# TUMFTM/RadarGNN

Measured on AMD Instinct MI355X. Metric: radar frames/sec (graph-build + GNN fwd), higher is better.
Workload: dtype f32 (dense layers: fp32 operands split into 2 f16 terms after an exact power-of-two pre-scale, 3 f16 MFMA products per fp32 product, fp32 accumulate -- more accurate than fp32 MFMA against float64, tests/test_gpu_f16x2.py; RGNN_NO_F16X2=1 selects 3 bf16 terms / 6 products, RGNN_LINEAR_FP32=1 v_mfma_; 1 GPU; C2: per GPU 64 RadarScenes-shaped frames x 3000 pts, radius graph r=1.0, node feats [rcs,velocity_vector,time_index,degree], edge feats [relative_position], 4-layer MPNNConv [224,224,128,64] + emb MLPs + both heads, train-mode BatchNorm, max aggr; frames_per_gpu=64, points_per_gpu=192000, edges_per_gpu=799078, ranks_in_process_group=1

## Files before the change

radargnn_amd/csrc/mpnn_tiles.hip:

```cpp
#include "common.h"
#include <stdlib.h>
#include <type_traits>

namespace {

constexpr int MT_THREADS = 256;
constexpr int MT_WAVES = MT_THREADS / 64;
constexpr int MT_QUEUE_INTS = 8 * 16;

typedef float mt_f32x16 __attribute__((ext_vector_type(16)));
typedef __bf16 mt_bf16x8 __attribute__((ext_vector_type(8)));
typedef unsigned int mt_u32x4 __attribute__((ext_vector_type(4)));

__global__ __launch_bounds__(256) void k_tiles_zero_empty(const int32_t* __restrict__ rowptr, const int32_t* __restrict__ order,
                                                         int64_t n, int d, float* __restrict__ out, int64_t ldo) {
  const int lane = threadIdx.x & 63;
  const int64_t p = (int64_t)blockIdx.x * MT_WAVES + (threadIdx.x >> 6);
  if (p >= n || rowptr[p + 1] != rowptr[p]) return;
  const int64_t node = order ? order[p] : p;
  for (int c = lane; c < d; c += 64) out[node * ldo + c] = 0.f;
}

__device__ __forceinline__ void mt_split3(float x, unsigned& t1, unsigned& t2, unsigned& t3) {
  t1 = __float_as_uint(x) & 0xffff0000u;
  const float r = x - __uint_as_float(t1);
  t2 = __float_as_uint(r) & 0xffff0000u;
  const float r2 = r - __uint_as_float(t2);
  t3 = __float_as_uint(r2) & 0xffff0000u;
}
__device__ __forceinline__ unsigned mt_pack(unsigned lo, unsigned hi) { return (lo >> 16) | hi; }
__device__ __forceinline__ void mt_split_row(const float (&x)[8], mt_u32x4& p1, mt_u32x4& p2, mt_u32x4& p3) {
  unsigned t1[8], t2[8], t3[8];
#pragma unroll
  for (int k = 0; k < 8; k++) mt_split3(x[k], t1[k], t2[k], t3[k]);
  p1 = mt_u32x4{mt_pack(t1[0], t1[1]), mt_pack(t1[2], t1[3]), mt_pack(t1[4], t1[5]), mt_pack(t1[6], t1[7])};
  p2 = mt_u32x4{mt_pack(t2[0], t2[1]), mt_pack(t2[2], t2[3]), mt_pack(t2[4], t2[5]), mt_pack(t2[6], t2[7])};
  p3 = mt_u32x4{mt_pack(t3[0], t3[1]), mt_pack(t3[2], t3[3]), mt_pack(t3[4], t3[5]), mt_pack(t3[6], t3[7])};
}

}

namespace {

constexpr int WN_SLOTS = 512;
constexpr int WN_THREADS = 256;
typedef int wn_i32x4 __attribute__((ext_vector_type(4)));

struct WinParams {
  const float* p_bias;
  const float* Q; int ldq4; int q_bytes;
  const mt_u32x4* wplanes;
  const float* ea; int de; int ea_vec;
  int n_win;
  const int32_t* n_win_dev;
  const int32_t* plan; int plan_bytes;
  int off_misc;
  int off_eid;
  int off_lrow;
  int off_urow;
  int off_tgt;
  int32_t* queue;
  int d; int n_ct;
  float* out; int ldo4; int o_bytes;
  float* out_absmax;
  int abl;
};

__device__ __forceinline__ void wn_dma16(wn_i32x4 rsrc, int voff, int soff, unsigned lds_base) {
  asm volatile(
      "s_mov_b32 m0, %3\n\t"
      "s_nop 0\n\t"
      "buffer_load_dwordx4 %0, %1, %2 offen lds"
      :
      : "v"(voff), "s"(rsrc), "s"(soff), "s"(lds_base)
      : "memory");
}

__global__ __launch_bounds__(256) void k_win_wplanes(const float* __restrict__ We, int ldwe, int de, int d, int n_ct, const float* __restrict__ p_bias,
                                                     mt_u32x4* __restrict__ planes) {
  const int c = blockIdx.x * blockDim.x + threadIdx.x;
  if (c >= n_ct * 32) return;
  float w[8];
#pragma unroll
  for (int k = 0; k < 8; k++) w[k] = (c < d && k < de) ? We[(int64_t)c * ldwe + k] : 0.f;
  mt_u32x4 p1, p2, p3;
  mt_split_row(w, p1, p2, p3);
  mt_u32x4* t = planes + (c >> 5) * 128 + (c & 31);
  t[0] = p1; t[32] = p2; t[64] = p3;
  t[96] = mt_u32x4{__float_as_uint((p_bias != nullptr && c < d) ? p_bias[c] : 0.f), 0u, 0u, 0u};
}

constexpr int WN_PAD = 4;
constexpr int WN_GPT = 16 / WN_PAD;
constexpr int WN_GPS = 64 / WN_PAD;
constexpr int WN_TMAX = 512 / WN_PAD;
static_assert(WN_PAD == 2 || WN_PAD == 4, "segments are padded to 2 or 4 slots");
constexpr int WN_UMAX = 176;
constexpr int WN_ROWBUF = WN_UMAX * 128;

__device__ __forceinline__ void wn_wait_leaving(int n) {
  switch (n) {
#define WN_W(N) case N: asm volatile("s_waitcnt vmcnt(" #N ")" ::: "memory"); break;
    WN_W(1) WN_W(2) WN_W(3) WN_W(4) WN_W(5) WN_W(6) WN_W(7) WN_W(8) WN_W(9) WN_W(10) WN_W(11) WN_W(12) WN_W(13) WN_W(14) WN_W(15) WN_W(16)
    WN_W(17) WN_W(18) WN_W(19) WN_W(20) WN_W(21) WN_W(22) WN_W(23) WN_W(24) WN_W(25) WN_W(26) WN_W(27) WN_W(28) WN_W(29) WN_W(30) WN_W(31) WN_W(32)
#undef WN_W
    default: asm volatile("s_waitcnt vmcnt(0)" ::: "memory"); break;
  }
}

constexpr bool WN_WARM = false;
constexpr int WN_BBUF = 32 * 64;

constexpr int WN_DESC = 2 * WN_UMAX * 4 + 2048 + 512 + 8 * WN_GPS * 4 + 64;
static_assert((2 * WN_UMAX * 128 + 2 * 32 * 64 + WN_DESC + 16 + 511) / 512 * 512 * 3 <= 160 * 1024, "k_mpnn_win: LDS of three work-groups per CU");
constexpr int WN_LDS = 2 * WN_ROWBUF + 2 * WN_BBUF + WN_DESC + 16;

template <bool AMAX>
__global__ __launch_bounds__(WN_THREADS) __attribute__((amdgpu_waves_per_eu(3, 3))) void k_mpnn_win(const WinParams p) {
  extern __shared__ __attribute__((aligned(16))) char smem[];
  char* bstage = smem + 2 * WN_ROWBUF;
  int* urowtab = (int*)(bstage + 2 * WN_BBUF);
  int* eidtab = urowtab + 2 * WN_UMAX;
  const uint8_t* lrowtab = (const uint8_t*)(eidtab + 512);
  int* tgttab = eidtab + 512 + 128;
  int* misctab = tgttab + 8 * WN_GPS;
  int* bcast = misctab + 16;
  const unsigned rows_lds = (unsigned)(uintptr_t)(__attribute__((address_space(3))) char*)smem;
  const unsigned b_lds = rows_lds + 2 * WN_ROWBUF;
  const unsigned desc_lds = b_lds + 2 * WN_BBUF;
  const int tid = threadIdx.x, lane = tid & 63, wave = __builtin_amdgcn_readfirstlane(tid >> 6), half = lane >> 5, col = lane & 31, col4 = col * 4;
  const int xcd = blockIdx.x & 7;
  const int n_win = min(p.n_win, __builtin_amdgcn_readfirstlane(p.n_win_dev[0]));
  const int i_lo = (int)((int64_t)n_win * xcd / 8), i_hi = (int)((int64_t)n_win * (xcd + 1) / 8);
  int32_t* ticket = p.queue + xcd * 16;
  wn_i32x4 rq, rw, rp;
  {
    const uint64_t a = (uint64_t)p.Q;
    rq.x = __builtin_amdgcn_readfirstlane((int)(uint32_t)a);
    rq.y = __builtin_amdgcn_readfirstlane((int)(uint32_t)((a >> 32) & 0xffff));
    rq.z = __builtin_amdgcn_readfirstlane(p.q_bytes);
    rq.w = 0x00020000;
    const uint64_t b = (uint64_t)p.wplanes;
    rw.x = __builtin_amdgcn_readfirstlane((int)(uint32_t)b);
    rw.y = __builtin_amdgcn_readfirstlane((int)(uint32_t)((b >> 32) & 0xffff));
    rw.z = __builtin_amdgcn_readfirstlane(p.n_ct * WN_BBUF);
    rw.w = 0x00020000;
    const uint64_t c = (uint64_t)p.plan;
    rp.x = __builtin_amdgcn_readfirstlane((int)(uint32_t)c);
    rp.y = __builtin_amdgcn_readfirstlane((int)(uint32_t)((c >> 32) & 0xffff));
    rp.z = __builtin_amdgcn_readfirstlane(p.plan_bytes);
    rp.w = 0x00020000;
  }
  const __amdgpu_buffer_rsrc_t ro = __builtin_amdgcn_make_buffer_rsrc((void*)p.out, (short)0, p.o_bytes, 0x00020000);
  const int rA = lane & 31, hA = (rA >> 2) & 1, iA = ((rA >> 3) << 2) | (rA & 3);
  const int my_stream = 2 * wave + half;
  float amax = 0.f;
  float ninf = -INFINITY;
  asm volatile("" : "+v"(ninf));

  auto desc_dma = [&](const int w, const int up) {
    if (wave == 0) {
      if (lane < WN_UMAX / 4) wn_dma16(rp, lane * 16, __builtin_amdgcn_readfirstlane(p.off_urow + w * (WN_UMAX * 4)),
                                       (unsigned)__builtin_amdgcn_readfirstlane((int)(desc_lds + up * (WN_UMAX * 4))));
    } else if (wave == 1) {
      wn_dma16(rp, lane * 16, __builtin_amdgcn_readfirstlane(p.off_eid + w * 2048), desc_lds + 8 * WN_UMAX);
      wn_dma16(rp, lane * 16, __builtin_amdgcn_readfirstlane(p.off_eid + w * 2048 + 1024), desc_lds + 8 * WN_UMAX + 1024);
    } else if (wave == 2) {
      if (lane < 32) wn_dma16(rp, lane * 16, __builtin_amdgcn_readfirstlane(p.off_lrow + w * 512), desc_lds + 8 * WN_UMAX + 2048);
    } else {
      if (lane < 2 * WN_GPS) wn_dma16(rp, lane * 16, __builtin_amdgcn_readfirstlane(p.off_tgt + w * (32 * WN_GPS)), desc_lds + 8 * WN_UMAX + 2560);
      if (lane < 4) wn_dma16(rp, lane * 16, __builtin_amdgcn_readfirstlane(p.off_misc + w * 64), desc_lds + 8 * WN_UMAX + 2560 + 32 * WN_GPS);
    }
  };
  auto stage = [&](const int ct, const int st, const int up, const int nU8) {
    const unsigned base = rows_lds + st * WN_ROWBUF;
    const int* ut = urowtab + up * WN_UMAX;
    for (int k = wave; k < nU8; k += 4)
      wn_dma16(rq, (int)__umul24((unsigned)ut[8 * k + (lane >> 3)], (unsigned)p.ldq4) + (lane & 7) * 16, __builtin_amdgcn_readfirstlane(ct * 128),
               (unsigned)__builtin_amdgcn_readfirstlane((int)(base + k * 1024)));
    if (wave == 1) {
      const unsigned bb = b_lds + st * WN_BBUF;
      wn_dma16(rw, lane * 16, __builtin_amdgcn_readfirstlane(ct * WN_BBUF), (unsigned)__builtin_amdgcn_readfirstlane((int)bb));
      wn_dma16(rw, lane * 16 + 1024, __builtin_amdgcn_readfirstlane(ct * WN_BBUF), (unsigned)__builtin_amdgcn_readfirstlane((int)(bb + 1024)));
    }
  };

  if (tid == 0) { bcast[0] = i_lo + atomicAdd(ticket, 1); bcast[1] = i_lo + atomicAdd(ticket, 1); }
  __syncthreads();
  int win = bcast[0];
  int up = 0;
  int gp = 0;
  bool staged = false;
  if (win < i_hi) desc_dma(win, 0);
  asm volatile("s_waitcnt vmcnt(0)" ::: "memory");
  __syncthreads();
  for (;;) {
    if (win >= i_hi) {
      if (tid == 0) {
        const int wgs = (int)(gridDim.x >> 3);
        if (atomicAdd(ticket + 1, 1) == wgs - 1) { ticket[0] = 0; ticket[1] = 0; }
      }
      break;
    }
    const int nxt = bcast[1];
    const int nU = misctab[0];
    const int nU8 = (nU + 7) >> 3;
    int nt = 0;
    unsigned endbits = 0, anyend = 0, endA = 0, endB = 0;
    mt_u32x4 a1[4], a2[4], a3[4];
    int aoff[4][16];
    int tv = 0;
    if (nU != 0) {
      tv = tgttab[my_stream * WN_GPS + (lane & (WN_GPS - 1))] * p.ldo4;
      const uint8_t* m8 = (const uint8_t*)(misctab + 1);
      nt = max((int)m8[2 * wave], (int)m8[2 * wave + 1]);
      const uint8_t* e4 = m8 + 8 + my_stream * 4;
      endbits = (unsigned)e4[0] | ((unsigned)e4[1] << WN_GPT) | ((unsigned)e4[2] << (2 * WN_GPT)) | ((unsigned)e4[3] << (3 * WN_GPT));
      endA = (unsigned)__builtin_amdgcn_readlane((int)endbits, 0); endB = (unsigned)__builtin_amdgcn_readlane((int)endbits, 32);
      anyend = endA | endB;
#pragma unroll
      for (int t = 0; t < 4; t++) {
        const int e = eidtab[(2 * wave + hA) * 64 + t * 16 + iA];
        float z[8];
        if (p.ea_vec) {
          const float4 mine = *(const float4*)(p.ea + (int64_t)e * 8 + half * 4);
          const float4 other = make_float4(__shfl_xor(mine.x, 32, 64), __shfl_xor(mine.y, 32, 64), __shfl_xor(mine.z, 32, 64), __shfl_xor(mine.w, 32, 64));
          const float4 lo = half ? other : mine, hi = half ? mine : other;
          z[0] = lo.x; z[1] = lo.y; z[2] = lo.z; z[3] = lo.w; z[4] = hi.x; z[5] = hi.y; z[6] = hi.z; z[7] = hi.w;
        } else {
#pragma unroll
          for (int k = 0; k < 8; k++) z[k] = (k < p.de) ? p.ea[(int64_t)e * p.de + k] : 0.f;
        }
        mt_u32x4 t3;
        mt_split_row(z, a1[t], a2[t], t3);
        a3[t] = half ? a1[t] : t3;
      }
      const mt_u32x4* lt = (const mt_u32x4*)(lrowtab + my_stream * 64);
#pragma unroll
      for (int t = 0; t < 4; t++) {
        const mt_u32x4 w4 = lt[t];
#pragma unroll
        for (int i = 0; i < 16; i++) {
          const unsigned w = w4[i >> 2];
          const unsigned r = (i & 3) == 3 ? (w >> 24) : ((w >> (8 * (i & 3))) & 0xffu);
          aoff[t][i] = (int)(rows_lds + (r << 7)) + col4;
          asm volatile("" : "+v"(aoff[t][i]));
        }
      }
    }
    __syncthreads();
    if (tid == 0) bcast[1] = i_lo + atomicAdd(ticket, 1);
    if (nU == 0) {
      if (nxt < i_hi) desc_dma(nxt, up ^ 1);
      asm volatile("s_waitcnt vmcnt(0)" ::: "memory");
      __syncthreads();
      win = nxt; up ^= 1; staged = false;
      continue;
    }
    const int nst = __builtin_popcount(anyend & ((nt >= 4) ? (WN_GPT == 8 ? 0xffffffffu : 0xffffu) : ((1u << (WN_GPT * nt)) - 1u)));
    if (!staged) stage(0, gp, up, nU8);
    bool staged_next = false;

    auto tile_pass = [&](const int ct, auto stage_c) {
      constexpr int ST = decltype(stage_c)::value;
      if (ct == 0 || (p.abl & 1)) asm volatile("s_waitcnt vmcnt(0)" ::: "memory");
      else wn_wait_leaving(nst);
      __syncthreads();
      if (ct == 0 && nxt < i_hi) desc_dma(nxt, up ^ 1);
      if (ct + 1 < p.n_ct) {
        if (!(p.abl & 1)) stage(ct + 1, ST ^ 1, up, nU8);
      } else if (ct > 0 && nxt < i_hi && !(p.abl & 1)) {
        const int nUn = misctab[0];
        if (nUn != 0) { stage(0, ST ^ 1, up ^ 1, (nUn + 7) >> 3); staged_next = true; }
      }
      const mt_u32x4* bl = (const mt_u32x4*)(bstage + ST * WN_BBUF);
      const mt_u32x4 bxc = bl[(half ? 32 : 0) + col], byc = bl[(half ? 64 : 0) + col];
      const float biasc = __uint_as_float(bl[96 + col].x);
      const int voffc = (ct * 32 + col < p.d) ? col4 : 0x7ffffff0;
      const float ninf_l = ninf;
      const __amdgpu_buffer_rsrc_t ro_l = ro;
      float rn = -INFINITY;
      asm volatile("" : "+v"(tv), "+s"(endA), "+s"(endB), "+s"(anyend));
#pragma unroll
      for (int t = 0; t < 4; t++) {
        if (t < nt && !(p.abl & 2)) {
          mt_f32x16 c;
#pragma unroll
          for (int i = 0; i < 16; i++) c[i] = *(const __attribute__((address_space(3))) float*)(uintptr_t)(unsigned)(aoff[t][i] + ST * WN_ROWBUF);
          c = __builtin_amdgcn_mfma_f32_32x32x16_bf16(__builtin_bit_cast(mt_bf16x8, a3[t]), __builtin_bit_cast(mt_bf16x8, byc), c, 0, 0, 0);
          c = __builtin_amdgcn_mfma_f32_32x32x16_bf16(__builtin_bit_cast(mt_bf16x8, a2[t]), __builtin_bit_cast(mt_bf16x8, bxc), c, 0, 0, 0);
          c = __builtin_amdgcn_mfma_f32_32x32x16_bf16(__builtin_bit_cast(mt_bf16x8, a1[t]), __builtin_bit_cast(mt_bf16x8, bxc), c, 0, 0, 0);
#pragma unroll
          for (int g = 0; g < WN_GPT; g++) {
            rn = __builtin_fmaxf(__builtin_fmaxf(rn, c[WN_PAD * g]), c[WN_PAD * g + 1]);
            if (WN_PAD == 4) rn = __builtin_fmaxf(__builtin_fmaxf(rn, c[WN_PAD * g + 2]), c[WN_PAD * g + 3]);
            if ((anyend >> (WN_GPT * t + g)) & 1u) {
              const int k = WN_GPT * t + g;
              const float v = rn + biasc;
              const unsigned long long mA = ((endA >> k) & 1u) ? 0xffffffffull : 0ull, mB = ((endB >> k) & 1u) ? 0xffffffff00000000ull : 0ull;
              const int soA = __builtin_amdgcn_readlane(tv, k) + ct * 128, soB = __builtin_amdgcn_readlane(tv, 32 + k) + ct * 128;
              if (!(p.abl & 4)) {
                const int off = (half ? soB : soA) + voffc;
                asm volatile("s_mov_b64 exec, %3\n\tbuffer_store_dword %0, %1, %2, 0 offen nt\n\ts_mov_b64 exec, -1"
                             : : "v"(v), "v"(off), "s"(ro_l), "s"(mA | mB) : "memory");
              }
              if (AMAX) amax = fmaxf(amax, fabsf(v));
              const unsigned long long m64 = mA | mB;
              asm volatile("v_cndmask_b32_e64 %0, %0, %1, %2" : "+v"(rn) : "v"(ninf_l), "s"(m64));
            }
          }
        }
      }
    };
    float amax_full = 0.f;
    for (int ct = 0; ct < p.n_ct; ct++) {
      const bool partial = AMAX && (ct + 1) * 32 > p.d;
      if (partial) { amax_full = amax; amax = 0.f; }
      if ((gp + ct) & 1) tile_pass(ct, std::integral_constant<int, 1>());
      else tile_pass(ct, std::integral_constant<int, 0>());
      if (partial) amax = fmaxf(amax_full, (ct * 32 + col < p.d) ? amax : 0.f);
    }
    if (p.n_ct < 2) {
      asm volatile("s_waitcnt vmcnt(0)" ::: "memory");
      __syncthreads();
    }
    gp = (gp + p.n_ct) & 1;
    win = nxt; up ^= 1; staged = staged_next;
  }
  if (AMAX) {
#pragma unroll
    for (int o = 32; o > 0; o >>= 1) amax = fmaxf(amax, __shfl_xor(amax, o, 64));
    if (lane == 0)
      atomicMax((unsigned int*)p.out_absmax + ((blockIdx.x * 4 + wave) & (RGNN_BOUND_SLOTS - 1)), __float_as_uint(amax));
  }
}

constexpr int WN_BIG = 64;

constexpr int WN_SEG = 512;
struct WinPlanLayout {
  int n_win, n_seg;
  int64_t off_assign, off_segcnt, off_segbase, off_wend, off_pdeg, off_wstart, off_left, off_leftcnt, off_queue, off_misc, off_tgt, off_eid, off_lrow, off_urow,
      off_wplanes, total_ints;
};
WinPlanLayout win_layout(int64_t n, int64_t n_edges) {
  WinPlanLayout L;
  L.n_seg = (int)((n + WN_SEG - 1) / WN_SEG);
  L.n_win = (int)((n_edges + 3 * n) / 256 + L.n_seg + 2);
  int64_t o = 16;
  auto take = [&](int64_t ints) { const int64_t at = o; o = (o + ints + 15) / 16 * 16; return at; };
  L.off_assign = take(n + 1); L.off_segcnt = take(L.n_seg + 1); L.off_segbase = take(L.n_seg + 2);
  L.off_wend = take(L.n_win + 1);
  L.off_pdeg = take(n + 1); L.off_wstart = take(L.n_win + 1); L.off_left = take(n + 1); L.off_leftcnt = take(4);
  L.off_queue = take(MT_QUEUE_INTS); L.off_misc = take(16 * (int64_t)L.n_win);
  L.off_tgt = take(8 * WN_GPS * (int64_t)L.n_win); L.off_eid = take(512 * (int64_t)L.n_win); L.off_lrow = take(128 * (int64_t)L.n_win);
  L.off_urow = take(WN_UMAX * (int64_t)L.n_win); L.off_wplanes = take(16 * 64 * 32);
  L.total_ints = o;
  return L;
}

__global__ __launch_bounds__(256) void k_win_pdeg(const int32_t* __restrict__ rowptr, int64_t n, int32_t* __restrict__ pdeg,
                                                 int32_t* __restrict__ left, int32_t* __restrict__ leftcnt, int32_t* __restrict__ queue) {
  const int64_t p = (int64_t)blockIdx.x * blockDim.x + threadIdx.x;
  if (p < MT_QUEUE_INTS) queue[p] = 0;
  if (p > n) return;
  if (p == n) { pdeg[p] = 0; return; }
  const int d = rowptr[p + 1] - rowptr[p];
  const int pd = (d + WN_PAD - 1) & ~(WN_PAD - 1);
  if (pd > WN_BIG) left[atomicAdd(leftcnt, 1)] = (int32_t)p;
  pdeg[p] = (pd > WN_BIG) ? 0 : pd;
}
__global__ __launch_bounds__(64) void k_win_greedy(const int32_t* __restrict__ pdeg, int64_t n, int32_t* __restrict__ assign,
                                                  int32_t* __restrict__ segcnt) {
  __shared__ int spd[WN_SEG];
  __shared__ int sas[WN_SEG];
  const int seg = blockIdx.x, lane = threadIdx.x;
  const int64_t p0 = (int64_t)seg * WN_SEG;
  const int cnt = (int)min((int64_t)WN_SEG, n - p0);
  for (int i = lane; i < cnt; i += 64) spd[i] = pdeg[p0 + i];
  __syncthreads();
  {
    int fill = 0;
    int win = 0, any = 0;
    for (int ib = 0; ib < cnt; ib += 64) {
      const int mine_pd = (ib + lane < cnt) ? spd[ib + lane] : 0;
      int mine_as = -1;
      const int nb = min(64, cnt - ib);
      for (int j = 0; j < nb; j++) {
        const int pd = __builtin_amdgcn_readlane(mine_pd, j);
        if (pd == 0) continue;
        const unsigned long long fits = __ballot(lane < 8 && fill + pd <= 64);
        int b = 0;
        if (fits == 0) { win++; fill = 0; }
        else b = __builtin_ctzll(fits);
        const int off = __builtin_amdgcn_readlane(fill, b);
        if (lane == b) fill += pd;
        any = 1;
        if (lane == j) mine_as = (win << 16) | (b * 64 + off);
      }
      if (ib + lane < cnt) sas[ib + lane] = mine_as;
    }
    if (lane == 0) segcnt[seg] = any ? win + 1 : 0;
  }
  __syncthreads();
  for (int i = lane; i < cnt; i += 64) assign[p0 + i] = sas[i];
}
__global__ __launch_bounds__(1024) void k_win_segbase(const int32_t* __restrict__ segcnt, int n_seg, int32_t* __restrict__ segbase) {
  __shared__ int part[1024];
  const int t = threadIdx.x;
  const int per = (n_seg + 1023) / 1024;
  int sum = 0;
  for (int i = t * per; i < min(n_seg, (t + 1) * per); i++) sum += segcnt[i];
  part[t] = sum;
  __syncthreads();
  for (int o = 1; o < 1024; o <<= 1) {
    const int v = t >= o ? part[t - o] : 0;
    __syncthreads();
    part[t] += v;
    __syncthreads();
  }
  int run = part[t] - sum;
  for (int i = t * per; i < min(n_seg, (t + 1) * per); i++) { segbase[i] = run; run += segcnt[i]; }
  if (t == 1023) segbase[n_seg] = part[1023];
}
__global__ __launch_bounds__(256) void k_win_starts(const int32_t* __restrict__ assign, const int32_t* __restrict__ segbase, int64_t n, int n_seg,
                                                   int n_win, int32_t* __restrict__ wstart, int32_t* __restrict__ wend) {
  const int64_t p = (int64_t)blockIdx.x * blockDim.x + threadIdx.x;
  if (p >= n) return;
  const int a = assign[p];
  if (a < 0) return;
  const int seg = (int)(p / WN_SEG);
  const int w = segbase[seg] + (a >> 16);
  if (w >= n_win) return;
  if ((a & 0xffff) == 0) wstart[w] = (int32_t)p;
  atomicMax(&wend[w], (int32_t)p + 1);
}

__global__ __launch_bounds__(256) void k_win_pack(const int32_t* __restrict__ rowptr, const int32_t* __restrict__ src,
                                                 const int32_t* __restrict__ order, const int32_t* __restrict__ pdeg,
                                                 const int32_t* __restrict__ assign, const int32_t* __restrict__ segbase,
                                                 const int32_t* __restrict__ wstart, const int32_t* __restrict__ wend, int n_win,
                                                 int32_t* __restrict__ misc_out, int32_t* __restrict__ tgt_out,
                                                 int32_t* __restrict__ eid_out, uint8_t* __restrict__ lrow_out, int32_t* __restrict__ urow_out,
                                                 int32_t* __restrict__ left, int32_t* __restrict__ leftcnt) {
  __shared__ int s_src[4][512];
  __shared__ int s_key[4][1024];
  __shared__ int s_val[4][1024];
  __shared__ short s_assign[4][WN_TMAX];
  __shared__ int s_pos[4][WN_TMAX];
  __shared__ int s_pd[4][WN_TMAX];
  __shared__ int s_e0[4][WN_TMAX];
  __shared__ int s_misc[4][16];
  __shared__ int s_end[4][32];
  const int lane = threadIdx.x & 63, wv = threadIdx.x >> 6;
  const int w = blockIdx.x * 4 + wv;
  if (w >= n_win) return;
  const int p1 = wend[w], p0 = p1 > 0 ? wstart[w] : 0;
  int* ssrc = s_src[wv]; int* skey = s_key[wv]; int* sval = s_val[wv]; short* sas = s_assign[wv]; int* spos = s_pos[wv]; int* spd = s_pd[wv]; int* se0 = s_e0[wv]; int* misc = s_misc[wv]; int* send = s_end[wv];
  const int64_t wb = (int64_t)w * 512;
  if (p1 == 0) {
    if (lane < 16) misc_out[(int64_t)w * 16 + lane] = 0;
    return;
  }
  for (int i = lane; i < 512; i += 64) { ssrc[i] = -1; eid_out[wb + i] = 0; lrow_out[wb + i] = 0; }
  for (int i = lane; i < 1024; i += 64) skey[i] = -1;
  for (int i = lane; i < 8 * WN_GPS; i += 64) tgt_out[(int64_t)w * (8 * WN_GPS) + i] = 0;
  if (lane < 32) send[lane] = 0;
  if (lane == 0) misc[9] = 0;
  __builtin_amdgcn_s_waitcnt(0);
  __builtin_amdgcn_wave_barrier();
  for (int pb = p0; pb < p1; pb += 64) {
    const int p = pb + lane;
    const int a = p < p1 ? assign[p] : -1;
    const bool mine = a >= 0 && segbase[p / WN_SEG] + (a >> 16) == w;
    const unsigned long long m = __ballot(mine);
    const int base = misc[9];
    const int j = base + __popcll(m & ((1ull << lane) - 1ull));
    if (mine) {
      if (j < WN_TMAX) { spos[j] = p; spd[j] = pdeg[p]; se0[j] = rowptr[p]; sas[j] = (short)(a & 0xffff); }
      else left[atomicAdd(leftcnt, 1)] = p;
    }
    __builtin_amdgcn_s_waitcnt(0);
    __builtin_amdgcn_wave_barrier();
    if (lane == 0) misc[9] = min(base + __popcll(m), WN_TMAX);
    __builtin_amdgcn_s_waitcnt(0);
    __builtin_amdgcn_wave_barrier();
  }
  const int cnt = misc[9];
  if (lane < 8) misc[lane] = 0;
  __builtin_amdgcn_s_waitcnt(0);
  __builtin_amdgcn_wave_barrier();
  for (int i = lane; i < cnt; i += 64) atomicMax(&misc[sas[i] >> 6], (sas[i] & 63) + spd[i]);
  for (int i = lane; i < cnt; i += 64) {
    const int at = sas[i], p = spos[i], e0 = se0[i], pd = spd[i];
    const int d = rowptr[p + 1] - e0;
    for (int q = 0; q < pd; q++) {
      const int e = e0 + min(q, d - 1);
      eid_out[wb + at + q] = e;
      ssrc[at + q] = src[e];
    }
    const int gi = ((at & 63) + pd - WN_PAD) / WN_PAD, b = at >> 6;
    atomicOr(&send[b * 4 + gi / WN_GPT], 1 << (gi % WN_GPT));
    tgt_out[(int64_t)w * (8 * WN_GPS) + b * WN_GPS + gi] = order ? order[p] : p;
  }
  __builtin_amdgcn_s_waitcnt(0);
  __builtin_amdgcn_wave_barrier();
  if (lane == 0) misc[8] = 0;
  for (int i = lane; i < 512; i += 64) {
    const int s_ = ssrc[i];
    if (s_ < 0) continue;
    unsigned h = ((unsigned)s_ * 2654435761u) >> 22;
    for (;;) {
      const int prev = atomicCAS(&skey[h], -1, s_);
      if (prev == -1 || prev == s_) break;
      h = (h + 1) & 1023;
    }
  }
  __builtin_amdgcn_s_waitcnt(0);
  __builtin_amdgcn_wave_barrier();
  for (int i = lane; i < 1024; i += 64)
    if (skey[i] >= 0) sval[i] = atomicAdd(&misc[8], 1);
  __builtin_amdgcn_s_waitcnt(0);
  __builtin_amdgcn_wave_barrier();
  const int nU = misc[8];
  if (nU > WN_UMAX) {
    for (int i = lane; i < cnt; i += 64) left[atomicAdd(leftcnt, 1)] = spos[i];
    if (lane < 16) misc_out[(int64_t)w * 16 + lane] = 0;
    return;
  }
  for (int i = lane; i < 1024; i += 64)
    if (skey[i] >= 0) urow_out[(int64_t)w * WN_UMAX + sval[i]] = skey[i];
  for (int i = lane; i < 512; i += 64) {
    const int s_ = ssrc[i];
    if (s_ < 0) continue;
    unsigned h = ((unsigned)s_ * 2654435761u) >> 22;
    while (skey[h] != s_) h = (h + 1) & 1023;
    lrow_out[wb + i] = (uint8_t)sval[h];
  }
  if (lane < 8 && nU + lane < ((nU + 7) & ~7)) urow_out[(int64_t)w * WN_UMAX + nU + lane] = 0;
  uint8_t* m8 = (uint8_t*)(misc_out + (int64_t)w * 16);
  if (lane == 0) misc_out[(int64_t)w * 16] = nU;
  if (lane < 8) m8[4 + lane] = (uint8_t)((misc[lane] + 15) >> 4);
  if (lane < 32) m8[12 + lane] = (uint8_t)send[lane];
  if (lane < 5) m8[44 + 4 * lane] = 0, m8[45 + 4 * lane] = 0, m8[46 + 4 * lane] = 0, m8[47 + 4 * lane] = 0;
}

__global__ __launch_bounds__(256) void k_win_leftover(const float* __restrict__ p_bias, const float* __restrict__ Q, int64_t ldq,
                                                     const float* __restrict__ We, int ldwe, const float* __restrict__ ea, int de,
                                                     const int32_t* __restrict__ rowptr, const int32_t* __restrict__ src,
                                                     const int32_t* __restrict__ order, const int32_t* __restrict__ left,
                                                     const int32_t* __restrict__ leftcnt, int d, float* __restrict__ out, int64_t ldo,
                                                     float* __restrict__ out_absmax) {
  const int lane = threadIdx.x & 63, wv = threadIdx.x >> 6;
  const int n_left = *leftcnt;
  if (n_left == 0) return;
  float amax = 0.f;
  for (int c0 = 0; c0 < d; c0 += 512) {
    const int cw = c0 + 128 * wv;
    if (cw >= d) continue;
    float w[2][8];
    bool ok[2];
#pragma unroll
    for (int j = 0; j < 2; j++) {
      const int c = cw + 64 * j + lane;
      ok[j] = c < d;
#pragma unroll
      for (int k = 0; k < 8; k++) w[j][k] = (ok[j] && k < de) ? We[(int64_t)c * ldwe + k] : 0.f;
    }
    for (int64_t i = blockIdx.x; i < n_left; i += gridDim.x) {
      const int p = left[i];
      const int e0 = rowptr[p], e1 = rowptr[p + 1];
      const int64_t node = order ? order[p] : p;
      float m[2] = {-INFINITY, -INFINITY};
      for (int eb = e0; eb < e1; eb += 64) {
        const int el = min(eb + lane, e1 - 1);
        const int my_src = src[el];
        float my_z[8];
#pragma unroll
        for (int k = 0; k < 8; k++) my_z[k] = k < de ? ea[(int64_t)el * de + k] : 0.f;
        const int nb = min(64, e1 - eb);
        for (int q = 0; q < nb; q += 8) {
          float v[8][2];
          int jj[8];
#pragma unroll
          for (int u = 0; u < 8; u++) {
            jj[u] = min(q + u, nb - 1);
            const int64_t r = (int64_t)__builtin_amdgcn_readlane(my_src, jj[u]) * ldq + cw + lane;
#pragma unroll
            for (int j = 0; j < 2; j++) v[u][j] = ok[j] ? Q[r + 64 * j] : 0.f;
          }
#pragma unroll
          for (int u = 0; u < 8; u++) {
            float z[8];
#pragma unroll
            for (int k = 0; k < 8; k++) z[k] = __builtin_bit_cast(float, __builtin_amdgcn_readlane(__builtin_bit_cast(int, my_z[k]), jj[u]));
#pragma unroll
            for (int j = 0; j < 2; j++) {
#pragma unroll
              for (int k = 0; k < 8; k++) v[u][j] = __builtin_fmaf(w[j][k], z[k], v[u][j]);
              m[j] = fmaxf(m[j], v[u][j]);
            }
          }
        }
      }
#pragma unroll
      for (int j = 0; j < 2; j++) {
        if (!ok[j]) continue;
        const int c = cw + 64 * j + lane;
        const float o = m[j] + (p_bias ? p_bias[c] : 0.f);
        out[node * ldo + c] = o;
        amax = fmaxf(amax, fabsf(o));
      }
    }
  }
  if (out_absmax != nullptr) {
#pragma unroll
    for (int o = 32; o > 0; o >>= 1) amax = fmaxf(amax, __shfl_xor(amax, o, 64));
    if (lane == 0 && amax > 0.f)
      atomicMax((unsigned int*)out_absmax + ((blockIdx.x * 4 + wv) & (RGNN_BOUND_SLOTS - 1)), __float_as_uint(amax));
  }
}

}

extern "C" int64_t rgnn_mpnn_win_plan_ints(int64_t n, int64_t n_edges) { return win_layout(n, n_edges).total_ints; }
extern "C" void rgnn_mpnn_win_plan_counters(int64_t n, int64_t n_edges, int64_t* leftover_word, int64_t* windows_word) {
  const WinPlanLayout L = win_layout(n, n_edges);
  *leftover_word = L.off_leftcnt;
  *windows_word = L.off_segbase + L.n_seg;
}

extern "C" int rgnn_mpnn_win_plan(const int32_t* rowptr_t, const int32_t* src_sorted, const int32_t* node_order, int64_t n, int64_t n_edges,
                                  int32_t* plan, rgnn_stream_t stream) {
  RGNN_CHECK_ARG(rowptr_t && plan && n >= 0 && n_edges >= 0, "bad arguments");
  RGNN_CHECK_ARG(n_edges == 0 || src_sorted, "null src_sorted");
  RGNN_CHECK_ARG((((uintptr_t)plan) & 15) == 0, "plan must be 16-byte aligned");
  if (n == 0) return RGNN_OK;
  const WinPlanLayout L = win_layout(n, n_edges);
  hipStream_t s = (hipStream_t)stream;
  hipMemsetAsync(plan + L.off_leftcnt, 0, 16, s);
  hipLaunchKernelGGL(k_win_pdeg, dim3(rgnn_blocks(n + 1 > MT_QUEUE_INTS ? n + 1 : MT_QUEUE_INTS, 256)), dim3(256), 0, s, rowptr_t, n, plan + L.off_pdeg,
                     plan + L.off_left, plan + L.off_leftcnt, plan + L.off_queue);
  hipMemsetAsync(plan + L.off_wend, 0, 4 * (size_t)(L.n_win + 1), s);
  hipLaunchKernelGGL(k_win_greedy, dim3(L.n_seg), dim3(64), 0, s, (const int32_t*)(plan + L.off_pdeg), n, plan + L.off_assign, plan + L.off_segcnt);
  hipLaunchKernelGGL(k_win_segbase, dim3(1), dim3(1024), 0, s, (const int32_t*)(plan + L.off_segcnt), L.n_seg, plan + L.off_segbase);
  hipLaunchKernelGGL(k_win_starts, dim3(rgnn_blocks(n, 256)), dim3(256), 0, s, (const int32_t*)(plan + L.off_assign),
                     (const int32_t*)(plan + L.off_segbase), n, L.n_seg, L.n_win, plan + L.off_wstart, plan + L.off_wend);
  hipLaunchKernelGGL(k_win_pack, dim3(rgnn_blocks(L.n_win, 4)), dim3(256), 0, s, rowptr_t, src_sorted, node_order,
                     (const int32_t*)(plan + L.off_pdeg), (const int32_t*)(plan + L.off_assign), (const int32_t*)(plan + L.off_segbase),
                     (const int32_t*)(plan + L.off_wstart), (const int32_t*)(plan + L.off_wend), L.n_win, plan + L.off_misc,
                     plan + L.off_tgt, plan + L.off_eid, (uint8_t*)(plan + L.off_lrow),
                     plan + L.off_urow, plan + L.off_left, plan + L.off_leftcnt);
  RGNN_CHECK_LAUNCH();
  return RGNN_OK;
}

extern "C" int64_t rgnn_mpnn_win_wplanes_bytes(int32_t d) { return d < 1 ? -1 : (int64_t)((d + 31) / 32) * WN_BBUF; }

extern "C" int rgnn_mpnn_win_wplanes(const float* We, int64_t ldwe, int32_t de, int32_t d, const float* p_bias, void* planes,
                                     rgnn_stream_t stream) {
  RGNN_CHECK_ARG(planes && d >= 1 && de >= 0 && de <= 8 && (de == 0 || We) && (((uintptr_t)planes) & 15) == 0, "bad arguments");
  const int n_ct = (d + 31) / 32;
  hipLaunchKernelGGL(k_win_wplanes, dim3(rgnn_blocks(n_ct * 32, 256)), dim3(256), 0, (hipStream_t)stream, We, (int)ldwe, de, d, n_ct, p_bias,
                     (mt_u32x4*)planes);
  RGNN_CHECK_LAUNCH();
  return RGNN_OK;
}

static int aggregate_win(const float* p_bias, const float* Q, int64_t ldq, const float* We, int64_t ldwe,
                         const float* edge_attr_sorted, int32_t de, const int32_t* rowptr_t, const int32_t* src_sorted,
                         const int32_t* node_order, int32_t* plan, int64_t n, int64_t n_edges, int32_t d, float* out,
                         int64_t ldo, int32_t flags, float* out_absmax, const void* wplanes, rgnn_stream_t stream) {
  if (n == 0) return RGNN_OK;
  RGNN_CHECK_ARG(Q && rowptr_t && plan && out && d >= 1, "bad arguments");
  RGNN_CHECK_ARG((flags & ~RGNN_MPNN_SKIP_EMPTY_ROWS) == 0, "unknown flags");
  RGNN_CHECK_ARG(de == 0 || ((We || wplanes) && edge_attr_sorted), "edge attributes given without weights");
  RGNN_CHECK_ARG((((uintptr_t)wplanes) & 15) == 0, "operand image not 16-byte aligned");
  const int64_t q_bytes = ((n - 1) * ldq + d) * 4, o_bytes = ((n - 1) * ldo + d) * 4;
  if (de > 8 || d > 2048 || n >= ((int64_t)1 << 24) || ldq * 4 >= ((int64_t)1 << 24) || q_bytes >= ((int64_t)1 << 31) ||
      o_bytes >= ((int64_t)1 << 31) || (ldq % 4) != 0 || (((uintptr_t)Q) & 15) != 0 || win_layout(n, n_edges).total_ints * 4 >= ((int64_t)1 << 31)) {
    rgnn_set_error("rgnn_mpnn_aggregate_win: shape not covered (de %d, d %d, n %lld, ldq %lld)", de, d, (long long)n, (long long)ldq);
    return RGNN_ERR_UNSUPPORTED;
  }
  hipStream_t s = (hipStream_t)stream;
  if (!(flags & RGNN_MPNN_SKIP_EMPTY_ROWS))
    hipLaunchKernelGGL(k_tiles_zero_empty, dim3(rgnn_blocks(n, MT_WAVES)), dim3(256), 0, s, rowptr_t, node_order, n, d, out, ldo);
  if (n_edges > 0) {
    const WinPlanLayout L = win_layout(n, n_edges);
    WinParams p;
    p.p_bias = p_bias; p.Q = Q; p.ldq4 = (int)(ldq * 4); p.q_bytes = (int)q_bytes;
    p.wplanes = wplanes ? (const mt_u32x4*)wplanes : (const mt_u32x4*)(plan + L.off_wplanes); p.ea = edge_attr_sorted; p.de = de;
    p.ea_vec = (de == 8 && (((uintptr_t)edge_attr_sorted) & 15) == 0) ? 1 : 0;
    p.n_win = L.n_win; p.n_win_dev = plan + L.off_segbase + L.n_seg;
    p.plan = plan; p.plan_bytes = (int)(L.total_ints * 4);
    p.off_misc = (int)(L.off_misc * 4); p.off_eid = (int)(L.off_eid * 4); p.off_lrow = (int)(L.off_lrow * 4); p.off_urow = (int)(L.off_urow * 4); p.off_tgt = (int)(L.off_tgt * 4);
    p.queue = plan + L.off_queue;
    p.d = d; p.n_ct = (d + 31) / 32; p.out = out; p.ldo4 = (int)(ldo * 4); p.o_bytes = (int)o_bytes; p.out_absmax = out_absmax;
    p.abl = RGNN_ENV("RGNN_MPNN_WIN_ABL") ? atoi(RGNN_ENV("RGNN_MPNN_WIN_ABL")) : 0;
    if (!wplanes)
      hipLaunchKernelGGL(k_win_wplanes, dim3(rgnn_blocks(p.n_ct * 32, 256)), dim3(256), 0, s, We, (int)ldwe, de, d, p.n_ct, p_bias,
                         (mt_u32x4*)(plan + L.off_wplanes));
    const size_t lds = WN_LDS;
    static RgnnOncePerDevice attr_once;
    if (attr_once.first()) {
      hipFuncSetAttribute((const void*)k_mpnn_win<true>, hipFuncAttributeMaxDynamicSharedMemorySize, (int)lds);
      hipFuncSetAttribute((const void*)k_mpnn_win<false>, hipFuncAttributeMaxDynamicSharedMemorySize, (int)lds);
    }
    static const int per_cu = RGNN_ENV("RGNN_MPNN_WIN_WG_PER_CU") ? atoi(RGNN_ENV("RGNN_MPNN_WIN_WG_PER_CU")) : 3;
    int64_t blocks = L.n_win;
    if (blocks > 256 * per_cu) blocks = 256 * per_cu;
    blocks = (blocks + 7) / 8 * 8;
    rgnn_prof_begin(s);
    if (out_absmax) hipLaunchKernelGGL((k_mpnn_win<true>), dim3((unsigned)blocks), dim3(WN_THREADS), lds, s, p);
    else hipLaunchKernelGGL((k_mpnn_win<false>), dim3((unsigned)blocks), dim3(WN_THREADS), lds, s, p);
    rgnn_prof_end(s);
    hipLaunchKernelGGL(k_win_leftover, dim3(2048), dim3(256), 0, s, p_bias, Q, ldq, We, (int)ldwe, edge_attr_sorted, de, rowptr_t, src_sorted,
                       node_order, (const int32_t*)(plan + L.off_left), (const int32_t*)(plan + L.off_leftcnt), d, out, ldo, out_absmax);
  }
  RGNN_CHECK_LAUNCH();
  return RGNN_OK;
}

extern "C" int rgnn_mpnn_aggregate_win(const float* p_bias, const float* Q, int64_t ldq, const float* We, int64_t ldwe,
                                       const float* edge_attr_sorted, int32_t de, const int32_t* rowptr_t, const int32_t* src_sorted,
                                       const int32_t* node_order, int32_t* plan, int64_t n, int64_t n_edges, int32_t d, float* out,
                                       int64_t ldo, int32_t flags, float* out_absmax, rgnn_stream_t stream) {
  return aggregate_win(p_bias, Q, ldq, We, ldwe, edge_attr_sorted, de, rowptr_t, src_sorted, node_order, plan, n, n_edges, d, out, ldo, flags,
                       out_absmax, nullptr, stream);
}

extern "C" int rgnn_mpnn_aggregate_win_planes(const float* p_bias, const float* Q, int64_t ldq, const float* We, int64_t ldwe,
                                              const float* edge_attr_sorted, int32_t de, const int32_t* rowptr_t,
                                              const int32_t* src_sorted, const int32_t* node_order, int32_t* plan, int64_t n,
                                              int64_t n_edges, int32_t d, float* out, int64_t ldo, int32_t flags, float* out_absmax,
                                              const void* wplanes, rgnn_stream_t stream) {
  RGNN_CHECK_ARG(wplanes != nullptr, "null operand image");
  return aggregate_win(p_bias, Q, ldq, We, ldwe, edge_attr_sorted, de, rowptr_t, src_sorted, node_order, plan, n, n_edges, d, out, ldo, flags,
                       out_absmax, wplanes, stream);
}
```

Baseline: 32070 frames/s.

## Fuse window-plan degree, greedy packing and bounds into fewer kernels

Folds the padded-degree kernel into the greedy window-packing kernel and removes the per-node window start/end atomic kernel. The greedy kernel now records window bounds per segment directly, and the segment-base scan emits a window-to-segment map. The 8-slot fill search is rewritten as SWAR byte arithmetic on a packed 64-bit word instead of ballots. The intent is to cut launches, memsets and atomics in graph-plan construction, at the cost of fixed per-segment window tables and a serial loop in the single-block scan.

```diff
diff --git a/radargnn_amd/csrc/mpnn_tiles.hip b/radargnn_amd/csrc/mpnn_tiles.hip
--- a/radargnn_amd/csrc/mpnn_tiles.hip
+++ b/radargnn_amd/csrc/mpnn_tiles.hip
@@ -338,10 +338,13 @@
 constexpr int WN_BIG = 64;
 
 constexpr int WN_SEG = 512;
+constexpr int WN_SEGWIN = 128;
+static_assert(WN_SEG * WN_BIG / 264 + 1 <= WN_SEGWIN, "per-segment window tables too small");
+static_assert(WN_BIG == 64 && WN_SEG == 512, "the packed fill word and the eight 64-position blocks of k_win_greedy");
 struct WinPlanLayout {
   int n_win, n_seg;
-  int64_t off_assign, off_segcnt, off_segbase, off_wend, off_pdeg, off_wstart, off_left, off_leftcnt, off_queue, off_misc, off_tgt, off_eid, off_lrow, off_urow,
-      off_wplanes, total_ints;
+  int64_t off_assign, off_segcnt, off_segbase, off_wbounds, off_wseg, off_pdeg, off_left, off_leftcnt, off_queue, off_misc, off_tgt, off_eid, off_lrow,
+      off_urow, off_wplanes, total_ints;
 };
 WinPlanLayout win_layout(int64_t n, int64_t n_edges) {
   WinPlanLayout L;
@@ -350,62 +353,74 @@
   int64_t o = 16;
   auto take = [&](int64_t ints) { const int64_t at = o; o = (o + ints + 15) / 16 * 16; return at; };
   L.off_assign = take(n + 1); L.off_segcnt = take(L.n_seg + 1); L.off_segbase = take(L.n_seg + 2);
-  L.off_wend = take(L.n_win + 1);
-  L.off_pdeg = take(n + 1); L.off_wstart = take(L.n_win + 1); L.off_left = take(n + 1); L.off_leftcnt = take(4);
-  L.off_queue = take(MT_QUEUE_INTS); L.off_misc = take(16 * (int64_t)L.n_win);
+  L.off_wbounds = take(2 * WN_SEGWIN * (int64_t)L.n_seg); L.off_wseg = take(L.n_win + 1);
+  L.off_pdeg = take(n + 1); L.off_left = take(n + 1);
+  L.off_leftcnt = take(4); L.off_queue = take(MT_QUEUE_INTS);
+  L.off_misc = take(16 * (int64_t)L.n_win);
   L.off_tgt = take(8 * WN_GPS * (int64_t)L.n_win); L.off_eid = take(512 * (int64_t)L.n_win); L.off_lrow = take(128 * (int64_t)L.n_win);
   L.off_urow = take(WN_UMAX * (int64_t)L.n_win); L.off_wplanes = take(16 * 64 * 32);
   L.total_ints = o;
   return L;
 }
 
-__global__ __launch_bounds__(256) void k_win_pdeg(const int32_t* __restrict__ rowptr, int64_t n, int32_t* __restrict__ pdeg,
-                                                 int32_t* __restrict__ left, int32_t* __restrict__ leftcnt, int32_t* __restrict__ queue) {
-  const int64_t p = (int64_t)blockIdx.x * blockDim.x + threadIdx.x;
-  if (p < MT_QUEUE_INTS) queue[p] = 0;
-  if (p > n) return;
-  if (p == n) { pdeg[p] = 0; return; }
-  const int d = rowptr[p + 1] - rowptr[p];
-  const int pd = (d + WN_PAD - 1) & ~(WN_PAD - 1);
-  if (pd > WN_BIG) left[atomicAdd(leftcnt, 1)] = (int32_t)p;
-  pdeg[p] = (pd > WN_BIG) ? 0 : pd;
-}
-__global__ __launch_bounds__(64) void k_win_greedy(const int32_t* __restrict__ pdeg, int64_t n, int32_t* __restrict__ assign,
-                                                  int32_t* __restrict__ segcnt) {
-  __shared__ int spd[WN_SEG];
-  __shared__ int sas[WN_SEG];
+__global__ __launch_bounds__(64) void k_win_greedy(const int32_t* __restrict__ rowptr, int64_t n, int32_t* __restrict__ pdeg,
+                                                  int32_t* __restrict__ assign, int32_t* __restrict__ segcnt, int2* __restrict__ wbounds,
+                                                  int32_t* __restrict__ left, int32_t* __restrict__ leftcnt) {
   const int seg = blockIdx.x, lane = threadIdx.x;
   const int64_t p0 = (int64_t)seg * WN_SEG;
   const int cnt = (int)min((int64_t)WN_SEG, n - p0);
-  for (int i = lane; i < cnt; i += 64) spd[i] = pdeg[p0 + i];
+  if (seg == 0 && lane == 0) pdeg[n] = 0;
+  __shared__ int s_rep[WN_SEG];
+  int2 rows[WN_SEG / 64];
+#pragma unroll
+  for (int k = 0; k < WN_SEG / 64; k++) {
+    const int i = k * 64 + lane;
+    rows[k] = i < cnt ? make_int2(rowptr[p0 + i], rowptr[p0 + i + 1]) : make_int2(0, 0);
+  }
+#pragma unroll
+  for (int k = 0; k < WN_SEG / 64; k++) {
+    const int i = k * 64 + lane;
+    int pd = (rows[k].y - rows[k].x + WN_PAD - 1) & ~(WN_PAD - 1);
+    if (i < cnt) {
+      if (pd > WN_BIG) { left[atomicAdd(leftcnt, 1)] = (int32_t)(p0 + i); pd = 0; }
+      pdeg[p0 + i] = pd;
+    }
+    s_rep[i] = pd * 0x01010101;
+  }
   __syncthreads();
-  {
-    int fill = 0;
-    int win = 0, any = 0;
-    for (int ib = 0; ib < cnt; ib += 64) {
-      const int mine_pd = (ib + lane < cnt) ? spd[ib + lane] : 0;
-      int mine_as = -1;
-      const int nb = min(64, cnt - ib);
-      for (int j = 0; j < nb; j++) {
-        const int pd = __builtin_amdgcn_readlane(mine_pd, j);
-        if (pd == 0) continue;
-        const unsigned long long fits = __ballot(lane < 8 && fill + pd <= 64);
-        int b = 0;
-        if (fits == 0) { win++; fill = 0; }
-        else b = __builtin_ctzll(fits);
-        const int off = __builtin_amdgcn_readlane(fill, b);
-        if (lane == b) fill += pd;
-        any = 1;
-        if (lane == j) mine_as = (win << 16) | (b * 64 + off);
+  int2* wb = wbounds + (int64_t)seg * WN_SEGWIN;
+  unsigned long long room = 0x8080808080808080ull;
+  unsigned long long bit7 = 0x8080808080808080ull;
+  asm volatile("" : "+s"(bit7));
+  int word = 192 - (1 << 16), opened = 0;
+  for (int ib = 0; ib < cnt; ib += 64) {
+    const int mine_rep = s_rep[ib + lane];
+    int mine_as = -1;
+    int sel = lane;
+    asm volatile("" : "+v"(sel));
+    auto place = [&](int j) {
+      const unsigned rep = (unsigned)__builtin_amdgcn_readlane(mine_rep, j);
+      if (rep == 0) return;
+      unsigned long long fits = ((((unsigned long long)((unsigned)(room >> 32) - rep)) << 32) | ((unsigned)room - rep)) & bit7;
+      if (__builtin_expect(fits == 0, 0)) {
+        if (word >= 0 && word < (WN_SEGWIN << 16)) wb[word >> 16] = make_int2((int)p0 + opened, (int)p0 + ib + j);
+        word += 1 << 16; room = 0xc0c0c0c0c0c0c0c0ull; opened = ib + j; fits = 0x80;
       }
-      if (ib + lane < cnt) sas[ib + lane] = mine_as;
-    }
-    if (lane == 0) segcnt[seg] = any ? win + 1 : 0;
-  }
-  __syncthreads();
-  for (int i = lane; i < cnt; i += 64) assign[p0 + i] = sas[i];
-}
-__global__ __launch_bounds__(1024) void k_win_segbase(const int32_t* __restrict__ segcnt, int n_seg, int32_t* __restrict__ segbase) {
+      const int sh = __builtin_ctzll(fits) - 7;
+      const int level = (int)(room >> sh) & 0xff;
+      room -= (unsigned long long)(rep & 0xff) << sh;
+      if (sel == j) mine_as = word + sh * 8 - level;
+    };
+    for (int jb = 0; jb < 64; jb += 8) {
+      place(jb); place(jb + 1); place(jb + 2); place(jb + 3); place(jb + 4); place(jb + 5); place(jb + 6); place(jb + 7);
+    }
+    if (ib + lane < cnt) assign[p0 + ib + lane] = mine_as;
+  }
+  if (word >= 0 && word < (WN_SEGWIN << 16)) wb[word >> 16] = make_int2((int)p0 + opened, (int)p0 + cnt);
+  if (lane == 0) segcnt[seg] = (word >> 16) + 1;
+}
+__global__ __launch_bounds__(1024) void k_win_segbase(const int32_t* __restrict__ segcnt, int n_seg, int n_win, int32_t* __restrict__ segbase,
+                                                     int32_t* __restrict__ wseg) {
   __shared__ int part[1024];
   const int t = threadIdx.x;
   const int per = (n_seg + 1023) / 1024;
@@ -420,26 +435,20 @@
     __syncthreads();
   }
   int run = part[t] - sum;
-  for (int i = t * per; i < min(n_seg, (t + 1) * per); i++) { segbase[i] = run; run += segcnt[i]; }
+  for (int i = t * per; i < min(n_seg, (t + 1) * per); i++) {
+    const int c = segcnt[i];
+    segbase[i] = run;
+    for (int k = 0; k < c; k++)
+      if (run + k < n_win) wseg[run + k] = (i << 8) | k;
+    run += c;
+  }
   if (t == 1023) segbase[n_seg] = part[1023];
-}
-__global__ __launch_bounds__(256) void k_win_starts(const int32_t* __restrict__ assign, const int32_t* __restrict__ segbase, int64_t n, int n_seg,
-                                                   int n_win, int32_t* __restrict__ wstart, int32_t* __restrict__ wend) {
-  const int64_t p = (int64_t)blockIdx.x * blockDim.x + threadIdx.x;
-  if (p >= n) return;
-  const int a = assign[p];
-  if (a < 0) return;
-  const int seg = (int)(p / WN_SEG);
-  const int w = segbase[seg] + (a >> 16);
-  if (w >= n_win) return;
-  if ((a & 0xffff) == 0) wstart[w] = (int32_t)p;
-  atomicMax(&wend[w], (int32_t)p + 1);
 }
 
 __global__ __launch_bounds__(256) void k_win_pack(const int32_t* __restrict__ rowptr, const int32_t* __restrict__ src,
                                                  const int32_t* __restrict__ order, const int32_t* __restrict__ pdeg,
                                                  const int32_t* __restrict__ assign, const int32_t* __restrict__ segbase,
-                                                 const int32_t* __restrict__ wstart, const int32_t* __restrict__ wend, int n_win,
+                                                 const int32_t* __restrict__ wseg, const int2* __restrict__ wbounds, int n_seg, int n_win,
                                                  int32_t* __restrict__ misc_out, int32_t* __restrict__ tgt_out,
                                                  int32_t* __restrict__ eid_out, uint8_t* __restrict__ lrow_out, int32_t* __restrict__ urow_out,
                                                  int32_t* __restrict__ left, int32_t* __restrict__ leftcnt) {
@@ -455,7 +464,10 @@
   const int lane = threadIdx.x & 63, wv = threadIdx.x >> 6;
   const int w = blockIdx.x * 4 + wv;
   if (w >= n_win) return;
-  const int p1 = wend[w], p0 = p1 > 0 ? wstart[w] : 0;
+  const bool made = w < segbase[n_seg];
+  const int sk = made ? wseg[w] : 0;
+  const int2 bounds = made ? wbounds[(int64_t)(sk >> 8) * WN_SEGWIN + (sk & 0xff)] : make_int2(0, 0);
+  const int p0 = bounds.x, p1 = bounds.y;
   int* ssrc = s_src[wv]; int* skey = s_key[wv]; int* sval = s_val[wv]; short* sas = s_assign[wv]; int* spos = s_pos[wv]; int* spd = s_pd[wv]; int* se0 = s_e0[wv]; int* misc = s_misc[wv]; int* send = s_end[wv];
   const int64_t wb = (int64_t)w * 512;
   if (p1 == 0) {
@@ -472,7 +484,7 @@
   for (int pb = p0; pb < p1; pb += 64) {
     const int p = pb + lane;
     const int a = p < p1 ? assign[p] : -1;
-    const bool mine = a >= 0 && segbase[p / WN_SEG] + (a >> 16) == w;
+    const bool mine = a >= 0 && (a >> 16) == (sk & 0xff);
     const unsigned long long m = __ballot(mine);
     const int base = misc[9];
     const int j = base + __popcll(m & ((1ull << lane) - 1ull));
@@ -638,17 +650,14 @@
   if (n == 0) return RGNN_OK;
   const WinPlanLayout L = win_layout(n, n_edges);
   hipStream_t s = (hipStream_t)stream;
-  hipMemsetAsync(plan + L.off_leftcnt, 0, 16, s);
-  hipLaunchKernelGGL(k_win_pdeg, dim3(rgnn_blocks(n + 1 > MT_QUEUE_INTS ? n + 1 : MT_QUEUE_INTS, 256)), dim3(256), 0, s, rowptr_t, n, plan + L.off_pdeg,
-                     plan + L.off_left, plan + L.off_leftcnt, plan + L.off_queue);
-  hipMemsetAsync(plan + L.off_wend, 0, 4 * (size_t)(L.n_win + 1), s);
-  hipLaunchKernelGGL(k_win_greedy, dim3(L.n_seg), dim3(64), 0, s, (const int32_t*)(plan + L.off_pdeg), n, plan + L.off_assign, plan + L.off_segcnt);
-  hipLaunchKernelGGL(k_win_segbase, dim3(1), dim3(1024), 0, s, (const int32_t*)(plan + L.off_segcnt), L.n_seg, plan + L.off_segbase);
-  hipLaunchKernelGGL(k_win_starts, dim3(rgnn_blocks(n, 256)), dim3(256), 0, s, (const int32_t*)(plan + L.off_assign),
-                     (const int32_t*)(plan + L.off_segbase), n, L.n_seg, L.n_win, plan + L.off_wstart, plan + L.off_wend);
+  hipMemsetAsync(plan + L.off_leftcnt, 0, 4 * (size_t)(L.off_queue + MT_QUEUE_INTS - L.off_leftcnt), s);
+  hipLaunchKernelGGL(k_win_greedy, dim3(L.n_seg), dim3(64), 0, s, rowptr_t, n, plan + L.off_pdeg, plan + L.off_assign, plan + L.off_segcnt,
+                     (int2*)(plan + L.off_wbounds), plan + L.off_left, plan + L.off_leftcnt);
+  hipLaunchKernelGGL(k_win_segbase, dim3(1), dim3(1024), 0, s, (const int32_t*)(plan + L.off_segcnt), L.n_seg, L.n_win, plan + L.off_segbase,
+                     plan + L.off_wseg);
   hipLaunchKernelGGL(k_win_pack, dim3(rgnn_blocks(L.n_win, 4)), dim3(256), 0, s, rowptr_t, src_sorted, node_order,
                      (const int32_t*)(plan + L.off_pdeg), (const int32_t*)(plan + L.off_assign), (const int32_t*)(plan + L.off_segbase),
-                     (const int32_t*)(plan + L.off_wstart), (const int32_t*)(plan + L.off_wend), L.n_win, plan + L.off_misc,
+                     (const int32_t*)(plan + L.off_wseg), (const int2*)(plan + L.off_wbounds), L.n_seg, L.n_win, plan + L.off_misc,
                      plan + L.off_tgt, plan + L.off_eid, (uint8_t*)(plan + L.off_lrow),
                      plan + L.off_urow, plan + L.off_left, plan + L.off_leftcnt);
   RGNN_CHECK_LAUNCH();
```

New measurement: 32580 frames/s (median of 6 runs). 1.6% higher.
